# adolfogonzalez3/custom_envs

Hardware: AMD Instinct MI355X
Metric: vectorised env-steps/sec, Optimize-v0 @4096 envs, 1/2/4/8 MI355X vs host CPU (higher is better)
Workload: dtype f64; 1 GPU; Optimize-v0 softmax-regression 256x10 (P=20, obs 41), 4096 envs per GPU, B=N=256, 40-step episodes with in-kernel auto-reset, device-resident actions/outputs; envs_per_gpu=4096, global_envs=4096, n_rows=256, n_features=10, n_classes=2, batch_size=256, steps_per_launch=250, outputs=every step kept: a [250]-record slab per launch, parallelism=env-sharded x1 (no collective)

## Files before the change

custom_envs_amd/csrc/optimize_lr_persist.h:

```cpp
#pragma once

#include "optimize_lr_mfma.h"

namespace ce {

struct ManyArgs {
    int k;
    long long act_stride;
    long long out_step;
};

constexpr int kLpWaves = 4;
constexpr int kLpMaxTpw = 8;

#ifndef CE_LP_G4
#define CE_LP_G4 1
#endif
#ifndef CE_LP_G4_XF
#define CE_LP_G4_XF 1
#endif
#ifndef CE_LP_EPI_SLEEP
#define CE_LP_EPI_SLEEP 0
#endif
#ifndef CE_LP_ROW_PRIO
#define CE_LP_ROW_PRIO 3
#endif
#ifndef CE_LP_LOG_HEAD
#define CE_LP_LOG_HEAD 1
#endif
__host__ __device__ constexpr bool lp_g4(int nkf) { return CE_LP_G4 && nkf <= 3; }

__host__ __device__ constexpr int lp_tpw(int N, int W = kLpWaves) {
    const int per = ((N + 15) / 16 + W - 1) / W;
    return per <= 1 ? 1 : per <= 2 ? 2 : per <= 4 ? 4 : per <= 8 ? 8 : 0;
}
__host__ __device__ constexpr bool lp_pad(int N, int W = kLpWaves) {
    return N % 16 != 0 || (N + 15) / 16 != W * lp_tpw(N, W);
}

#ifdef CE_DIAG
#define LP_STAMP(k)                                                   \
    do {                                                              \
        __builtin_amdgcn_sched_barrier(0);                            \
        lp_st[k] = __builtin_amdgcn_s_memrealtime();                  \
        __builtin_amdgcn_sched_barrier(0);                            \
    } while (0)
#else
#define LP_STAMP(k) \
    do {            \
    } while (0)
#endif

template <int NKF, int TPW, bool PAD, int W>
__global__ __launch_bounds__(kWave * W) void optimize_lr_persist_kernel(StepArgs<double> a, ManyArgs m) {
    constexpr int BLK = kWave * W;
    constexpr int P_MAX = 2 * kLrMaxF;
    constexpr int TD = lr_tile_doubles(NKF);
    constexpr int PR = (kLrEnvs * P_MAX + BLK - 1) / BLK;
    constexpr int OSM = 2 * P_MAX + 4;
    constexpr int NG = TPW < 4 ? TPW : 4;
    __shared__ double red_s[2][W][4][kWave];
    __shared__ double red_l[2][W][kLrEnvs];
    __shared__ double red_h[2][W][kLrEnvs];
    __shared__ __attribute__((aligned(16))) float obs_s[2][kLrEnvs * OSM];
    __shared__ double tab_s[CE_LR_TEXP ? kLrExpTab : 1];

#ifdef CE_DIAG
    unsigned long long lp_st[8] = {0};
#endif
    LP_STAMP(0);
    const int tid = threadIdx.x;
    const int lane = tid & (kWave - 1);
    const int wave = __builtin_amdgcn_readfirstlane(tid >> 6);
    const int c = lane & 15, h = lane >> 4;
    const int E = a.E, F = a.F, P = 2 * F, N = a.N, B = a.B;
    const int OS = a.obs_stride, OL = a.obs_lo;
    const int e0 = blockIdx.x * kLrEnvs;
    const int e = e0 + c;
    const bool env_ok = e < E;
    const unsigned pbase = static_cast<unsigned>(env_ok ? e : 0) * P;
    const double *img = reinterpret_cast<const double *>(a.data);
    const int ntiles = (N + 15) / 16;

#if CE_LR_TEXP
    LrExpSlice<BLK> tslice;
    tslice.load(img + static_cast<unsigned>(ntiles) * TD + kLrMaxF, tid);
#endif
    unsigned ioff[NKF];
    double2 wv[NKF], w0v[NKF];
    float2 av[NKF];
#if CE_LR_NOCLAMP
    double xm[NKF];
    const double *colmax = img + static_cast<unsigned>(ntiles) * TD;
#endif
#pragma unroll
    for (int k = 0; k < NKF; ++k) {
        const int f = 4 * k + h;
        ioff[k] = pbase + (f < F ? 2 * f : 0);
        wv[k] = *reinterpret_cast<const double2 *>(a.W + ioff[k]);
        w0v[k] = *reinterpret_cast<const double2 *>(a.W0 + ioff[k]);
        av[k] = *reinterpret_cast<const float2 *>(a.act + ioff[k]);
#if CE_LR_NOCLAMP
        xm[k] = colmax[f];
#endif
    }
    double xf[TPW][NKF], xg[TPW][4];
    unsigned vmask = 0;
#pragma unroll
    for (int i = 0; i < TPW; ++i) {
        const int t = wave + W * i;
        const bool live = !PAD || t < ntiles;
        const double *ti = img + static_cast<unsigned>(live ? t : 0) * TD;
#pragma unroll
        for (int k = 0; k < NKF; ++k) xf[i][k] = live ? ti[k * kWave + lane] : 0.0;
#pragma unroll
        for (int q = 0; q < 4; ++q) xg[i][q] = live ? ti[(NKF + q) * kWave + lane] : 0.0;
        if constexpr (PAD) {
            const int2 ya = reinterpret_cast<const int2 *>(ti + (NKF + 4) * kWave)[lane];
            const int2 yb = reinterpret_cast<const int2 *>(ti + (NKF + 5) * kWave)[lane];
            const int ys[4] = {ya.x, ya.y, yb.x, yb.y};
#pragma unroll
            for (int q = 0; q < 4; ++q) vmask |= (live && ys[q] >= 0 ? 1u : 0u) << (4 * i + q);
        }
    }
    int step_c = a.step[env_ok ? e : 0];
    const int np_ = kLrEnvs * P;
    const int pmul = (65536 + P - 1) / P;
    int pj[PR], pp[PR], step_p[PR];
    bool prole[PR];
    unsigned gi[PR];
    double g_prev[PR], rG[PR];
#pragma unroll
    for (int r = 0; r < PR; ++r) {
        const int i = tid + r * BLK;
        pj[r] = (i * pmul) >> 16;
        pp[r] = i - pj[r] * P;
        prole[r] = i < np_ && e0 + pj[r] < E;
        gi[r] = static_cast<unsigned>(prole[r] ? e0 + pj[r] : 0) * P + (prole[r] ? pp[r] : 0);
        g_prev[r] = a.G[gi[r]];
        step_p[r] = a.step[prole[r] ? e0 + pj[r] : 0];
    }
    const int sj = tid - (BLK - kLrEnvs);
    const bool srole = sj >= 0 && e0 + sj < E;
    const unsigned es = srole ? e0 + sj : 0;
    double lprev = a.L[es];
    int step_s = a.step[es];
#if CE_LR_TEXP
    tslice.store(tab_s, tid);
    __syncthreads();
#endif
    const double dB = static_cast<double>(B), rB = a.inv_B;
    double rL = rcp_newton2(lprev + 0.1);
#pragma unroll
    for (int r = 0; r < PR; ++r) rG[r] = rcp_newton2(fabs(g_prev[r]) + 1.0);
    if (OL == 0)
        for (int i = tid; i < kLrEnvs * OS; i += BLK) {
            const int j = i / OS, p = i - j * OS;
            if (p < P) obs_s[0][i] = obs_s[1][i] = 0.0f;
        }

    double wd[NKF];
    auto margins = [&]() {
#pragma unroll
        for (int k = 0; k < NKF; ++k) {
            const int f = 4 * k + h;
            const double w0 = wv[k].x - static_cast<double>(av[k].x);
            const double w1 = wv[k].y - static_cast<double>(av[k].y);
            wv[k] = double2{w0, w1};
            wd[k] = f < F ? w0 - w1 : 0.0;
        }
    };
    margins();
#ifdef CE_DIAG
    asm volatile("s_waitcnt vmcnt(0)" ::: "memory");
#endif
    LP_STAMP(1);

    constexpr int QC = 4;
    auto forward = [&](const double (&xv)[NKF]) {
        lr_d4 u = {0.0, 0.0, 0.0, 0.0};
#pragma unroll
        for (int k = 0; k < NKF; ++k) u = __builtin_amdgcn_mfma_f64_16x16x4f64(xv[k], wd[k], u, 0, 0, 0);
        return u;
    };
    const int nenv = E - e0 < kLrEnvs ? E - e0 : kLrEnvs;
    auto flush_obs = [&](int t) {
        float *ob = reinterpret_cast<float *>(reinterpret_cast<char *>(a.obs) + t * m.out_step) +
                    static_cast<unsigned>(e0) * OS;
        const float *src = obs_s[t & 1];
        const int nfl = nenv * OS, n4 = nfl >> 2;
        for (int i = tid; i < n4; i += BLK) {
            typedef float lp_f4 __attribute__((ext_vector_type(4)));
            const lp_f4 v = *reinterpret_cast<const lp_f4 *>(&src[4 * i]);
            asm volatile("global_store_dwordx4 %0, %1, off sc1" ::"v"(ob + 4 * i), "v"(v) : "memory");
        }
        for (int i = 4 * n4 + tid; i < nfl; i += BLK) lr_store(&ob[i], src[i]);
    };

    for (int t = 0; t < m.k; ++t) {
        const int buf = t & 1;
        float2 an[NKF];
        {
            const float *actn = a.act + (t + 1 < m.k ? (t + 1) * m.act_stride : 0);
#pragma unroll
            for (int k = 0; k < NKF; ++k) an[k] = *reinterpret_cast<const float2 *>(actn + ioff[k]);
        }
#if CE_LR_NOCLAMP
        double ub = 0.0;
#pragma unroll
        for (int k = 0; k < NKF; ++k) ub = fma(fabs(wd[k]), xm[k], ub);
        const int tier = lr_tier(ub);
#else
        const int tier = kLrClamped;
#endif
        lr_d4 sacc = {0.0, 0.0, 0.0, 0.0};
        double prod = 1.0, nlog = 0.0, umin = 1.0;
        unsigned miss = 0;
        auto rows = [&](auto tier_c) {
            constexpr int TIER = decltype(tier_c)::value;
#pragma unroll
            for (int g0 = 0; g0 < TPW; g0 += NG) {
                if (g0 > 0) {
                    nlog -= lr_log(prod, tab_s);
                    prod = 1.0;
                }
                lr_d4 u[NG];
#pragma unroll
                for (int i = 0; i < NG; ++i) u[i] = forward(xf[g0 + i]);
#pragma unroll
                for (int i = 0; i < NG; ++i) {
                    double qv[4];
                    static_assert(QC == 4, "the tile's four values go through the exp together");
                    double tx[QC];
                    bool valid[QC];
#pragma unroll
                    for (int j = 0; j < QC; ++j) {
                        if constexpr (TIER == kLrClamped) tx[j] = clamp_u(u[i][j]);
                        else tx[j] = u[i][j];
                        valid[j] = !PAD || ((vmask >> (4 * (g0 + i) + j)) & 1u);
                    }
                    lr_exp_neg<QC>(tx, tab_s);
                    if constexpr (TIER == kLrBatched) {
                        lr_post4(u[i], tx, valid, qv, prod, miss);
                    } else {
#pragma unroll
                        for (int j = 0; j < QC; ++j) lr_post(u[i][j], tx[j], valid[j], qv[j], prod, miss);
                    }
                    lr_tie4<TIER>(u[i], valid, umin);
#pragma unroll
                    for (int q = 0; q < 4; ++q)
                        sacc = __builtin_amdgcn_mfma_f64_16x16x4f64(xg[g0 + i][q], qv[q], sacc, 0, 0, 0);
                }
            }
        };
        lr_run_tier(tier, rows);
        int hits = 4 * TPW - lr_miss_count(miss);
        if (__any(umin < 0x1p-52)) {
#pragma unroll
            for (int i = 0; i < TPW; ++i) {
                const int tt = wave + W * i;
                if (tt >= ntiles) continue;
                const double *ti = img + static_cast<unsigned>(tt) * TD;
                const int2 ya = reinterpret_cast<const int2 *>(ti + (NKF + 4) * kWave)[lane];
                const int2 yb = reinterpret_cast<const int2 *>(ti + (NKF + 5) * kWave)[lane];
                const int yv[4] = {ya.x, ya.y, yb.x, yb.y};
                const lr_d4 uu = forward(xf[i]);
                double tx[4];
#pragma unroll
                for (int q = 0; q < 4; ++q) tx[q] = abs_clamp750(uu[q]);
                exp_neg_multi_clamped<4>(tx);
#pragma unroll
                for (int q = 0; q < 4; ++q)
                    if (yv[q] >= 0 && tx[q] == 1.0) hits += (yv[q] == 0 ? 1 : 0) - lr_hit(uu[q]);
            }
        }
        double lsum = nlog - lr_log(prod, tab_s);
        lsum = fold_pair<16>(lsum, lsum);
        lsum = fold_pair<32>(lsum, lsum);
        const double hsum = static_cast<double>(fold_env_lanes(hits));
#pragma unroll
        for (int r = 0; r < 4; ++r) red_s[buf][wave][r][lane] = sacc[r];
        if (lane < kLrEnvs) {
            red_l[buf][wave][lane] = lsum;
            red_h[buf][wave][lane] = hsum;
        }
        {
            const bool wipe = step_c + 1 >= a.max_steps && a.auto_reset;
            step_c = wipe ? 0 : step_c + 1;
#pragma unroll
            for (int k = 0; k < NKF; ++k)
                if (wipe) wv[k] = w0v[k];
            if (t + 1 < m.k) {
#pragma unroll
                for (int k = 0; k < NKF; ++k) av[k] = an[k];
                margins();
            }
        }
        __syncthreads();
#ifdef CE_DIAG
        if (t == 0) LP_STAMP(2);
        if (t == 1) LP_STAMP(3);
        if (t == m.k - 1) LP_STAMP(4);
#endif
        if (t > 0) flush_obs(t - 1);

        const long long ro = t * m.out_step;
        if (srole) {
            double lt = 0.0, ht = 0.0;
#pragma unroll
            for (int w = 0; w < W; ++w) {
                lt += red_l[buf][w][sj];
                ht += red_h[buf][w][sj];
            }
            const double loss = div_rcp(lt, dB, rB);
            const double acc = div_rcp(ht, dB, rB);
            const double lnew = div_rcp(loss - lprev, lprev + 0.1, rL);
            const int cur = step_s + 1;
            const bool wipe = cur >= a.max_steps && a.auto_reset;
            if (a.reward) lr_store(reinterpret_cast<float *>(reinterpret_cast<char *>(a.reward) + ro) + es,
                                   static_cast<float>(-loss));
            lr_store(reinterpret_cast<float *>(reinterpret_cast<char *>(a.objective) + ro) + es,
                     static_cast<float>(loss));
            lr_store(reinterpret_cast<float *>(reinterpret_cast<char *>(a.accuracy) + ro) + es,
                     static_cast<float>(acc));
            if (a.done) (reinterpret_cast<uint8_t *>(a.done) + ro)[es] = cur >= a.max_steps ? 1 : 0;
            lr_store(reinterpret_cast<int32_t *>(reinterpret_cast<char *>(a.episode_len) + ro) + es, cur);
            obs_s[buf][sj * OS + P - OL] = wipe ? 0.0f : static_cast<float>(lnew);
            lprev = wipe ? 0.0 : lnew;
            step_s = wipe ? 0 : cur;
            rL = rcp_newton2(lprev + 0.1);
        }
#pragma unroll
        for (int r = 0; r < PR; ++r) {
            if (!prole[r]) continue;
            const bool wipe = step_p[r] + 1 >= a.max_steps && a.auto_reset;
            const int f = pp[r] >> 1;
            double sf = 0.0;
#pragma unroll
            for (int w = 0; w < W; ++w) sf += red_s[buf][w][f >> 2][pj[r] + 16 * (f & 3)];
            const double g = div_rcp((pp[r] & 1) ? sf : -sf, dB, rB);
            const double gnew = div_rcp(g, fabs(g_prev[r]) + 1.0, rG[r]);
            obs_s[buf][pj[r] * OS + P + 1 + pp[r] - OL] = wipe ? 0.0f : static_cast<float>(gnew);
            g_prev[r] = wipe ? 0.0 : gnew;
            step_p[r] = wipe ? 0 : step_p[r] + 1;
            rG[r] = rcp_newton2(fabs(g_prev[r]) + 1.0);
        }
    }
    LP_STAMP(5);
    __syncthreads();
    if (m.k > 0) flush_obs(m.k - 1);
    if (wave == 0 && env_ok) {
#pragma unroll
        for (int k = 0; k < NKF; ++k)
            if (4 * k + h < F) {
                lr_store(a.W + ioff[k], wv[k].x);
                lr_store(a.W + ioff[k] + 1, wv[k].y);
            }
    }
#pragma unroll
    for (int r = 0; r < PR; ++r)
        if (prole[r]) lr_store(&a.G[gi[r]], g_prev[r]);
    if (srole) {
        lr_store(&a.L[es], lprev);
        lr_store(&a.step[es], step_s);
    }
#ifdef CE_DIAG
    asm volatile("s_waitcnt vmcnt(0)" ::: "memory");
    LP_STAMP(6);
    const int row = blockIdx.x * W + wave;
    if (row < E && lane < 8) a.diag[static_cast<size_t>(row) * 8 + lane] = lp_st[lane];
#endif
}


template <int NKF, int TPW, bool PAD>
__global__ __launch_bounds__(512) void optimize_lr_persist_ws_kernel(
    double *Wp, const float *actp, const unsigned char *datap, double *Gp, int32_t *stepp, double *Lp,
    unsigned efp, int Np, StepArgs<double> a, ManyArgs m) {
    constexpr int W = 4;
    constexpr int BLK = 512;
    constexpr int EB = BLK - kWave * W;
    constexpr int P_MAX = 2 * kLrMaxF;
    constexpr int TD = lr_tile_doubles(NKF);
    constexpr int PR = (kLrEnvs * P_MAX + EB - 1) / EB;
    constexpr int OSM = 2 * P_MAX + 4;
    constexpr int NG = TPW < 4 ? TPW : 4;
    __shared__ double red_s[2][W][4][kWave];
    __shared__ double red_l[2][W][kLrEnvs];
    __shared__ double red_h[2][W][kLrEnvs];
    __shared__ __attribute__((aligned(16))) float obs_s[2][kLrEnvs * OSM];
    constexpr bool G4 = lp_g4(NKF);
    constexpr int G4S = 14;
    __shared__ __attribute__((aligned(16))) double xgs[G4 ? 1 : W][G4 ? 1 : TPW][4][kWave];
    __shared__ __attribute__((aligned(16))) double xga[G4 ? W : 1][G4 ? TPW : 1][16][G4S];
    __shared__ double tab_s[CE_LR_TEXP ? kLrExpTab : 1];

#ifdef CE_DIAG
    unsigned long long lp_st[8] = {0};
#endif
    LP_STAMP(0);
    const int tid = threadIdx.x;
    const int lane = tid & (kWave - 1);
    const int wave = __builtin_amdgcn_readfirstlane(tid >> 6);
    const int c = lane & 15, h = lane >> 4;
    const int E = static_cast<int>(efp & 0xffffffu), F = static_cast<int>(efp >> 24), P = 2 * F, N = Np, B = a.B;
    const int OS = a.obs_stride, OL = a.obs_lo;
    const int e0 = blockIdx.x * kLrEnvs;
    const double *img = reinterpret_cast<const double *>(datap);
    const int ntiles = (N + 15) / 16;
    const int nenv = E - e0 < kLrEnvs ? E - e0 : kLrEnvs;

#if CE_LR_TEXP
    LrExpSlice<BLK> tslice;
    tslice.load(img + static_cast<unsigned>(ntiles) * TD + kLrMaxF, tid);
#endif
    if (wave < W) {
#if CE_LP_ROW_PRIO > 0
        __builtin_amdgcn_s_setprio(CE_LP_ROW_PRIO);
#endif
        const int e = e0 + c;
        const bool env_ok = e < E;
        const unsigned pbase = static_cast<unsigned>(env_ok ? e : 0) * P;
        unsigned ioff[NKF];
        double2 wv[NKF], w0v[NKF];
        float2 av[NKF];
#if CE_LR_NOCLAMP
        double xm[NKF];
        const double *colmax = img + static_cast<unsigned>(ntiles) * TD;
#endif
#pragma unroll
        for (int k = 0; k < NKF; ++k) {
            const int f = 4 * k + h;
            ioff[k] = pbase + (f < F ? 2 * f : 0);
            wv[k] = *reinterpret_cast<const double2 *>(Wp + ioff[k]);
            av[k] = *reinterpret_cast<const float2 *>(actp + ioff[k]);
#if CE_LR_NOCLAMP
            xm[k] = colmax[f];
#endif
        }
        double xf[TPW][NKF];
#pragma unroll
        for (int k = 0; k < NKF; ++k) w0v[k] = *reinterpret_cast<const double2 *>(a.W0 + ioff[k]);
        unsigned vmask = 0;
#pragma unroll
        for (int i = 0; i < TPW; ++i) {
            const int t = wave + W * i;
            const bool live = !PAD || t < ntiles;
            const double *ti = img + static_cast<unsigned>(live ? t : 0) * TD;
#pragma unroll
            for (int k = 0; k < NKF; ++k) xf[i][k] = live ? ti[k * kWave + lane] : 0.0;
            if constexpr (G4) {
#if CE_LP_G4_XF
                const int km = 4 * (c & 3) + h, j4 = c >> 2;
#pragma unroll
                for (int g = 0; g < NKF; ++g) xga[wave][i][km][j4 * NKF + g] = xf[i][g];
#else
                const int b4 = (lane >> 2) & 3, km = 4 * (lane >> 4) + (lane & 3);
#pragma unroll
                for (int q = 0; q < 4; ++q)
                    if (b4 < NKF) xga[wave][i][km][q * NKF + b4] = live ? ti[(NKF + q) * kWave + lane] : 0.0;
#endif
            } else {
#pragma unroll
                for (int q = 0; q < 4; ++q) xgs[wave][i][q][lane] = live ? ti[(NKF + q) * kWave + lane] : 0.0;
            }
            if constexpr (PAD) {
                const int2 ya = reinterpret_cast<const int2 *>(ti + (NKF + 4) * kWave)[lane];
                const int2 yb = reinterpret_cast<const int2 *>(ti + (NKF + 5) * kWave)[lane];
                const int ys[4] = {ya.x, ya.y, yb.x, yb.y};
#pragma unroll
                for (int q = 0; q < 4; ++q) vmask |= (live && ys[q] >= 0 ? 1u : 0u) << (4 * i + q);
            }
        }
        int step_c = stepp[env_ok ? e : 0];
#if CE_LR_TEXP
        tslice.store(tab_s, tid);
        __syncthreads();
#endif
        double wd[NKF];
        auto margins = [&]() {
#pragma unroll
            for (int k = 0; k < NKF; ++k) {
                const int f = 4 * k + h;
                const double w0 = wv[k].x - static_cast<double>(av[k].x);
                const double w1 = wv[k].y - static_cast<double>(av[k].y);
                wv[k] = double2{w0, w1};
                wd[k] = f < F ? w0 - w1 : 0.0;
            }
        };
        margins();
#ifdef CE_DIAG
        asm volatile("s_waitcnt vmcnt(0)" ::: "memory");
#endif
        LP_STAMP(1);
        constexpr int QC = 4;
        auto forward = [&](const double (&xv)[NKF]) {
            lr_d4 u = {0.0, 0.0, 0.0, 0.0};
#pragma unroll
            for (int k = 0; k < NKF; ++k) u = __builtin_amdgcn_mfma_f64_16x16x4f64(xv[k], wd[k], u, 0, 0, 0);
            return u;
        };
        for (int t = 0; t < m.k; ++t) {
            const int buf = t & 1;
            float2 an[NKF];
            {
                const float *actn = actp + (t + 1 < m.k ? (t + 1) * m.act_stride : 0);
#pragma unroll
                for (int k = 0; k < NKF; ++k) an[k] = *reinterpret_cast<const float2 *>(actn + ioff[k]);
            }
#if CE_LR_NOCLAMP
            double ub = 0.0;
#pragma unroll
            for (int k = 0; k < NKF; ++k) ub = fma(fabs(wd[k]), xm[k], ub);
            const int tier = lr_tier(ub);
#else
            const int tier = kLrClamped;
#endif
            lr_d4 sacc = {0.0, 0.0, 0.0, 0.0};
            double gacc[NKF];
#pragma unroll
            for (int g = 0; g < NKF; ++g) gacc[g] = 0.0;
            double prod = 1.0, nlog = 0.0, umin = 1.0;
            unsigned miss = 0;
            [[maybe_unused]] LrLogHead lhead = {};
            auto rows = [&](auto tier_c) {
                constexpr int TIER = decltype(tier_c)::value;
#pragma unroll
                for (int g0 = 0; g0 < TPW; g0 += NG) {
                    if (g0 > 0) {
                        nlog -= lr_log(prod, tab_s);
                        prod = 1.0;
                    }
                    lr_d4 u[NG];
#pragma unroll
                    for (int i = 0; i < NG; ++i) u[i] = forward(xf[g0 + i]);
#pragma unroll
                    for (int i = 0; i < NG; ++i) {
                        double gv[G4 ? 4 * NKF : 4];
                        if constexpr (G4) {
                            typedef double lp_d2 __attribute__((ext_vector_type(2)));
                            const lp_d2 *src = reinterpret_cast<const lp_d2 *>(
                                &xga[wave][g0 + i][4 * (lane >> 4) + (lane & 3)][0]);
#pragma unroll
                            for (int p2 = 0; p2 < 2 * NKF; ++p2) {
                                const lp_d2 v = src[p2];
                                gv[2 * p2] = v.x;
                                gv[2 * p2 + 1] = v.y;
                            }
                        } else {
#pragma unroll
                            for (int q = 0; q < 4; ++q) gv[q] = xgs[wave][g0 + i][q][lane];
                        }
                        double qv[4];
                        static_assert(QC == 4, "the tile's four values go through the exp together");
                        double tx[QC];
                        bool valid[QC];
#pragma unroll
                        for (int j = 0; j < QC; ++j) {
                            if constexpr (TIER == kLrClamped) tx[j] = clamp_u(u[i][j]);
                            else tx[j] = u[i][j];
                            valid[j] = !PAD || ((vmask >> (4 * (g0 + i) + j)) & 1u);
                        }
                        lr_exp_neg<QC>(tx, tab_s);
                        if constexpr (TIER == kLrBatched) {
                            lr_post4(u[i], tx, valid, qv, prod, miss);
                        } else {
#pragma unroll
                            for (int j = 0; j < QC; ++j)
                                lr_post(u[i][j], tx[j], valid[j], qv[j], prod, miss);
                        }
                        lr_tie4<TIER>(u[i], valid, umin);
#if CE_LP_LOG_HEAD
                        if (g0 + NG >= TPW && i == NG - 1) {
                            lhead = lr_log_head(prod, tab_s);
                            __builtin_amdgcn_sched_barrier(0);
                        }
#endif
                        if constexpr (G4) {
#pragma unroll
                            for (int q = 0; q < 4; ++q)
#pragma unroll
                                for (int g = 0; g < NKF; ++g)
                                    gacc[g] = __builtin_amdgcn_mfma_f64_4x4x4f64(gv[q * NKF + g], qv[q], gacc[g], 0, 0, 0);
                        } else {
#pragma unroll
                            for (int q = 0; q < 4; ++q)
                                sacc = __builtin_amdgcn_mfma_f64_16x16x4f64(gv[q], qv[q], sacc, 0, 0, 0);
                        }
                    }
                }
            };
            lr_run_tier(tier, rows);
            int hits = 4 * TPW - lr_miss_count(miss);
            if (__any(umin < 0x1p-52)) {
#pragma unroll
                for (int i = 0; i < TPW; ++i) {
                    const int tt = wave + W * i;
                    if (tt >= ntiles) continue;
                    const double *ti = img + static_cast<unsigned>(tt) * TD;
                    const int2 ya = reinterpret_cast<const int2 *>(ti + (NKF + 4) * kWave)[lane];
                    const int2 yb = reinterpret_cast<const int2 *>(ti + (NKF + 5) * kWave)[lane];
                    const int yv[4] = {ya.x, ya.y, yb.x, yb.y};
                    const lr_d4 uu = forward(xf[i]);
                    double tx[4];
#pragma unroll
                    for (int q = 0; q < 4; ++q) tx[q] = abs_clamp750(uu[q]);
                    exp_neg_multi_clamped<4>(tx);
#pragma unroll
                    for (int q = 0; q < 4; ++q)
                        if (yv[q] >= 0 && tx[q] == 1.0) hits += (yv[q] == 0 ? 1 : 0) - lr_hit(uu[q]);
                }
            }
#if CE_LP_LOG_HEAD
            double lsum = nlog - lr_log_tail(lhead);
#else
            double lsum = nlog - lr_log(prod, tab_s);
#endif
            lsum = fold_pair<16>(lsum, lsum);
            lsum = fold_pair<32>(lsum, lsum);
            const double hsum = static_cast<double>(fold_env_lanes(hits));
            if constexpr (G4) {
#pragma unroll
                for (int g = 0; g < NKF; ++g) red_s[buf][wave][g][lane] = gacc[g];
            } else {
#pragma unroll
                for (int r = 0; r < 4; ++r) red_s[buf][wave][r][lane] = sacc[r];
            }
            if (lane < kLrEnvs) {
                red_l[buf][wave][lane] = lsum;
                red_h[buf][wave][lane] = hsum;
            }
            {
                const bool wipe = step_c + 1 >= a.max_steps && a.auto_reset;
                step_c = wipe ? 0 : step_c + 1;
                if (__any(wipe)) {
#pragma unroll
                    for (int k = 0; k < NKF; ++k)
                        if (wipe) wv[k] = w0v[k];
                }
                if (t + 1 < m.k) {
#pragma unroll
                    for (int k = 0; k < NKF; ++k) av[k] = an[k];
                    margins();
                }
            }
#ifdef CE_DIAG
            if (t == 1) LP_STAMP(7);
#endif
            __syncthreads();
#ifdef CE_DIAG
            if (t == 0) LP_STAMP(2);
            if (t == 1) LP_STAMP(3);
            if (t == m.k - 1) LP_STAMP(4);
#endif
        }
        LP_STAMP(5);
        __syncthreads();
        if (wave == 0 && env_ok) {
#pragma unroll
            for (int k = 0; k < NKF; ++k)
                if (4 * k + h < F) {
                    lr_store(Wp + ioff[k], wv[k].x);
                    lr_store(Wp + ioff[k] + 1, wv[k].y);
                }
        }
    } else {
        const int te = tid - kWave * W;
        const int np_ = kLrEnvs * P;
        const int pmul = (65536 + P - 1) / P;
        int pj[PR], pp[PR], step_p[PR];
        bool prole[PR];
        unsigned gi[PR];
        double g_prev[PR], rG[PR];
#pragma unroll
        for (int r = 0; r < PR; ++r) {
            const int i = te + r * EB;
            pj[r] = (i * pmul) >> 16;
            pp[r] = i - pj[r] * P;
            prole[r] = i < np_ && e0 + pj[r] < E;
            gi[r] = static_cast<unsigned>(prole[r] ? e0 + pj[r] : 0) * P + (prole[r] ? pp[r] : 0);
            g_prev[r] = Gp[gi[r]];
            step_p[r] = stepp[prole[r] ? e0 + pj[r] : 0];
        }
        const int sj = te - (EB - kLrEnvs);
        const bool srole = sj >= 0 && e0 + sj < E;
        const unsigned es = srole ? e0 + sj : 0;
        double lprev = Lp[es];
        int step_s = stepp[es];
#if CE_LR_TEXP
        tslice.store(tab_s, tid);
#endif
        const double dB = static_cast<double>(B), rB = a.inv_B;
        double rL = rcp_newton2(lprev + 0.1);
#pragma unroll
        for (int r = 0; r < PR; ++r) rG[r] = rcp_newton2(fabs(g_prev[r]) + 1.0);
#if CE_LR_TEXP
        __syncthreads();
#endif
        auto flush_obs = [&](int t) {
            float *ob = reinterpret_cast<float *>(reinterpret_cast<char *>(a.obs) + t * m.out_step) +
                        static_cast<unsigned>(e0) * OS;
            const float *src = obs_s[t & 1];
            const int nfl = nenv * OS, n4 = nfl >> 2;
            for (int i = te; i < n4; i += EB) {
                typedef float lp_f4 __attribute__((ext_vector_type(4)));
                const lp_f4 v = *reinterpret_cast<const lp_f4 *>(&src[4 * i]);
                asm volatile("global_store_dwordx4 %0, %1, off sc1" ::"v"(ob + 4 * i), "v"(v) : "memory");
            }
            for (int i = 4 * n4 + te; i < nfl; i += EB) lr_store(&ob[i], src[i]);
        };
        if (OL == 0)
            for (int i = te; i < kLrEnvs * OS; i += EB) {
                const int j = i / OS, p = i - j * OS;
                if (p < P) obs_s[0][i] = obs_s[1][i] = 0.0f;
            }
        auto epi_steps = [&](auto pow2_c) {
            auto divB = [&](double x) {
                if constexpr (decltype(pow2_c)::value) return x * rB;
                else return div_rcp(x, dB, rB);
            };
            for (int t = 0; t < m.k; ++t) {
                const int buf = t & 1;
                __syncthreads();
#if CE_LP_EPI_SLEEP > 0
                __builtin_amdgcn_s_sleep(CE_LP_EPI_SLEEP);
#endif
    #ifdef CE_DIAG
                if (t == 1) LP_STAMP(2);
    #endif
                if (t > 0) flush_obs(t - 1);
                const long long ro = t * m.out_step;
                if (srole) {
                    double lt = 0.0, ht = 0.0;
    #pragma unroll
                    for (int w = 0; w < W; ++w) {
                        lt += red_l[buf][w][sj];
                        ht += red_h[buf][w][sj];
                    }
                    const double loss = divB(lt);
                    const double acc = divB(ht);
                    const double lnew = div_rcp(loss - lprev, lprev + 0.1, rL);
                    const int cur = step_s + 1;
                    const bool wipe = cur >= a.max_steps && a.auto_reset;
                    if (a.reward) lr_store(reinterpret_cast<float *>(reinterpret_cast<char *>(a.reward) + ro) + es,
                                           static_cast<float>(-loss));
                    lr_store(reinterpret_cast<float *>(reinterpret_cast<char *>(a.objective) + ro) + es,
                             static_cast<float>(loss));
                    lr_store(reinterpret_cast<float *>(reinterpret_cast<char *>(a.accuracy) + ro) + es,
                             static_cast<float>(acc));
                    if (a.done) (reinterpret_cast<uint8_t *>(a.done) + ro)[es] = cur >= a.max_steps ? 1 : 0;
                    lr_store(reinterpret_cast<int32_t *>(reinterpret_cast<char *>(a.episode_len) + ro) + es, cur);
                    float ol = static_cast<float>(lnew);
                    lprev = lnew;
                    step_s = cur;
                    if (__any(wipe)) {
                        if (wipe) {
                            ol = 0.0f;
                            lprev = 0.0;
                            step_s = 0;
                        }
                    }
                    obs_s[buf][sj * OS + P - OL] = ol;
                    rL = rcp_newton2(lprev + 0.1);
                }
    #pragma unroll
                for (int r = 0; r < PR; ++r) {
                    if (!prole[r]) continue;
                    const bool wipe = step_p[r] + 1 >= a.max_steps && a.auto_reset;
                    const int f = pp[r] >> 1;
                    double sf = 0.0;
    #pragma unroll
                    for (int w = 0; w < W; ++w) sf += red_s[buf][w][f >> 2][pj[r] + 16 * (f & 3)];
                    const double g = divB((pp[r] & 1) ? sf : -sf);
                    const double gnew = div_rcp(g, fabs(g_prev[r]) + 1.0, rG[r]);
                    float og = static_cast<float>(gnew);
                    g_prev[r] = gnew;
                    step_p[r] = step_p[r] + 1;
                    if (__any(wipe)) {
                        if (wipe) {
                            og = 0.0f;
                            g_prev[r] = 0.0;
                            step_p[r] = 0;
                        }
                    }
                    obs_s[buf][pj[r] * OS + P + 1 + pp[r] - OL] = og;
                    rG[r] = rcp_newton2(fabs(g_prev[r]) + 1.0);
                }
    #ifdef CE_DIAG
                if (t == 1) {
                    asm volatile("s_waitcnt vmcnt(0) lgkmcnt(0)" ::: "memory");
                    LP_STAMP(7);
                }
    #endif
            }
        };
        if ((B & (B - 1)) == 0) epi_steps(std::true_type{});
        else epi_steps(std::false_type{});
        __syncthreads();
        if (m.k > 0) flush_obs(m.k - 1);
#pragma unroll
        for (int r = 0; r < PR; ++r)
            if (prole[r]) lr_store(&Gp[gi[r]], g_prev[r]);
        if (srole) {
            lr_store(&Lp[es], lprev);
            lr_store(&stepp[es], step_s);
        }
    }
#ifdef CE_DIAG
    asm volatile("s_waitcnt vmcnt(0)" ::: "memory");
    LP_STAMP(6);
    const int row = blockIdx.x * 8 + wave;
    if (row < E && lane < 8) a.diag[static_cast<size_t>(row) * 8 + lane] = lp_st[lane];
#endif
}

}
```

Before: 1.785 billion env-steps/s.

## Hand weight-margin update to an epilogue wave via an LDS ring

Moves the per-step weight update (action subtraction, auto-reset wipe, margin/tier computation and final weight writeback) out of the four MFMA row waves into a dedicated epilogue wave. That wave precomputes wd and tier two steps ahead and passes them through a two-slot shared-memory ring. The row waves then only read wd from LDS each step, taking action loads and reset logic off their critical path. In exchange it adds LDS traffic and an extra barrier, and correctness now depends on the ring depth matching the per-step __syncthreads cadence.

```diff
diff --git a/custom_envs_amd/csrc/optimize_lr_persist.h b/custom_envs_amd/csrc/optimize_lr_persist.h
--- a/custom_envs_amd/csrc/optimize_lr_persist.h
+++ b/custom_envs_amd/csrc/optimize_lr_persist.h
@@ -28,7 +28,12 @@
 #ifndef CE_LP_LOG_HEAD
 #define CE_LP_LOG_HEAD 1
 #endif
+#ifndef CE_LP_WD_HANDOVER
+#define CE_LP_WD_HANDOVER 1
+#endif
 __host__ __device__ constexpr bool lp_g4(int nkf) { return CE_LP_G4 && nkf <= 3; }
+constexpr int kLpWdWave = 2;
+constexpr int kLpWdRing = 2;
 
 __host__ __device__ constexpr int lp_tpw(int N, int W = kLpWaves) {
     const int per = ((N + 15) / 16 + W - 1) / W;
@@ -394,6 +399,10 @@
     __shared__ __attribute__((aligned(16))) double xgs[G4 ? 1 : W][G4 ? 1 : TPW][4][kWave];
     __shared__ __attribute__((aligned(16))) double xga[G4 ? W : 1][G4 ? TPW : 1][16][G4S];
     __shared__ double tab_s[CE_LR_TEXP ? kLrExpTab : 1];
+#if CE_LP_WD_HANDOVER
+    __shared__ double wd_s[kLpWdRing][NKF][kWave];
+    __shared__ int tier_s[kLpWdRing];
+#endif
 
 #ifdef CE_DIAG
     unsigned long long lp_st[8] = {0};
@@ -418,6 +427,7 @@
 #if CE_LP_ROW_PRIO > 0
         __builtin_amdgcn_s_setprio(CE_LP_ROW_PRIO);
 #endif
+#if !CE_LP_WD_HANDOVER
         const int e = e0 + c;
         const bool env_ok = e < E;
         const unsigned pbase = static_cast<unsigned>(env_ok ? e : 0) * P;
@@ -438,9 +448,12 @@
             xm[k] = colmax[f];
 #endif
         }
+#endif
         double xf[TPW][NKF];
+#if !CE_LP_WD_HANDOVER
 #pragma unroll
         for (int k = 0; k < NKF; ++k) w0v[k] = *reinterpret_cast<const double2 *>(a.W0 + ioff[k]);
+#endif
         unsigned vmask = 0;
 #pragma unroll
         for (int i = 0; i < TPW; ++i) {
@@ -472,12 +485,19 @@
                 for (int q = 0; q < 4; ++q) vmask |= (live && ys[q] >= 0 ? 1u : 0u) << (4 * i + q);
             }
         }
+#if !CE_LP_WD_HANDOVER
         int step_c = stepp[env_ok ? e : 0];
+#endif
 #if CE_LR_TEXP
         tslice.store(tab_s, tid);
+#endif
+#if CE_LR_TEXP || CE_LP_WD_HANDOVER
         __syncthreads();
 #endif
         double wd[NKF];
+#if CE_LP_WD_HANDOVER
+        int slot = 0;
+#else
         auto margins = [&]() {
 #pragma unroll
             for (int k = 0; k < NKF; ++k) {
@@ -489,6 +509,7 @@
             }
         };
         margins();
+#endif
 #ifdef CE_DIAG
         asm volatile("s_waitcnt vmcnt(0)" ::: "memory");
 #endif
@@ -502,6 +523,16 @@
         };
         for (int t = 0; t < m.k; ++t) {
             const int buf = t & 1;
+#if CE_LP_WD_HANDOVER
+#pragma unroll
+            for (int k = 0; k < NKF; ++k) wd[k] = wd_s[slot][k][lane];
+#if CE_LR_NOCLAMP
+            const int tier = __builtin_amdgcn_readfirstlane(tier_s[slot]);
+#else
+            const int tier = kLrClamped;
+#endif
+            slot = slot == kLpWdRing - 1 ? 0 : slot + 1;
+#else
             float2 an[NKF];
             {
                 const float *actn = actp + (t + 1 < m.k ? (t + 1) * m.act_stride : 0);
@@ -515,6 +546,7 @@
             const int tier = lr_tier(ub);
 #else
             const int tier = kLrClamped;
+#endif
 #endif
             lr_d4 sacc = {0.0, 0.0, 0.0, 0.0};
             double gacc[NKF];
@@ -630,6 +662,7 @@
                 red_l[buf][wave][lane] = lsum;
                 red_h[buf][wave][lane] = hsum;
             }
+#if !CE_LP_WD_HANDOVER
             {
                 const bool wipe = step_c + 1 >= a.max_steps && a.auto_reset;
                 step_c = wipe ? 0 : step_c + 1;
@@ -644,6 +677,7 @@
                     margins();
                 }
             }
+#endif
 #ifdef CE_DIAG
             if (t == 1) LP_STAMP(7);
 #endif
@@ -656,6 +690,7 @@
         }
         LP_STAMP(5);
         __syncthreads();
+#if !CE_LP_WD_HANDOVER
         if (wave == 0 && env_ok) {
 #pragma unroll
             for (int k = 0; k < NKF; ++k)
@@ -664,6 +699,7 @@
                     lr_store(Wp + ioff[k] + 1, wv[k].y);
                 }
         }
+#endif
     } else {
         const int te = tid - kWave * W;
         const int np_ = kLrEnvs * P;
@@ -687,6 +723,76 @@
         const unsigned es = srole ? e0 + sj : 0;
         double lprev = Lp[es];
         int step_s = stepp[es];
+#if CE_LP_WD_HANDOVER
+        const bool wown = wave == W + kLpWdWave;
+        const int e = e0 + c;
+        const bool env_ok = e < E;
+        unsigned ioff[NKF];
+        double2 wv[NKF], w0v[NKF];
+        float2 an[NKF];
+        [[maybe_unused]] double xm[NKF];
+        int step_c = 0;
+        auto wd_wipe = [&]() {
+            const bool wipe = step_c + 1 >= a.max_steps && a.auto_reset;
+            step_c = wipe ? 0 : step_c + 1;
+            if (__any(wipe)) {
+#pragma unroll
+                for (int k = 0; k < NKF; ++k)
+                    if (wipe) wv[k] = w0v[k];
+            }
+        };
+        auto wd_emit = [&](int slot, const float2 (&av)[NKF]) {
+            double wd[NKF];
+#pragma unroll
+            for (int k = 0; k < NKF; ++k) {
+                const int f = 4 * k + h;
+                const double w0 = wv[k].x - static_cast<double>(av[k].x);
+                const double w1 = wv[k].y - static_cast<double>(av[k].y);
+                wv[k] = double2{w0, w1};
+                wd[k] = f < F ? w0 - w1 : 0.0;
+            }
+#if CE_LR_NOCLAMP
+            double ub = 0.0;
+#pragma unroll
+            for (int k = 0; k < NKF; ++k) ub = fma(fabs(wd[k]), xm[k], ub);
+            tier_s[slot] = lr_tier(ub);
+#endif
+#pragma unroll
+            for (int k = 0; k < NKF; ++k) wd_s[slot][k][lane] = wd[k];
+        };
+        auto act_load = [&](int s, float2 (&av)[NKF]) {
+            const float *acts = actp + s * m.act_stride;
+#pragma unroll
+            for (int k = 0; k < NKF; ++k) av[k] = *reinterpret_cast<const float2 *>(acts + ioff[k]);
+        };
+        if (wown) {
+            const unsigned pbase = static_cast<unsigned>(env_ok ? e : 0) * P;
+#if CE_LR_NOCLAMP
+            const double *colmax = img + static_cast<unsigned>(ntiles) * TD;
+#endif
+#pragma unroll
+            for (int k = 0; k < NKF; ++k) {
+                const int f = 4 * k + h;
+                ioff[k] = pbase + (f < F ? 2 * f : 0);
+                wv[k] = *reinterpret_cast<const double2 *>(Wp + ioff[k]);
+                w0v[k] = *reinterpret_cast<const double2 *>(a.W0 + ioff[k]);
+#if CE_LR_NOCLAMP
+                xm[k] = colmax[f];
+#endif
+            }
+            step_c = stepp[env_ok ? e : 0];
+            float2 a0[kLpWdRing][NKF];
+#pragma unroll
+            for (int s = 0; s < kLpWdRing; ++s)
+                if (s < m.k) act_load(s, a0[s]);
+            if (kLpWdRing < m.k) act_load(kLpWdRing, an);
+#pragma unroll
+            for (int s = 0; s < kLpWdRing; ++s) {
+                if (s > 0 && s <= m.k) wd_wipe();
+                if (s < m.k) wd_emit(s, a0[s]);
+            }
+        }
+#endif
 #if CE_LR_TEXP
         tslice.store(tab_s, tid);
 #endif
@@ -694,7 +800,7 @@
         double rL = rcp_newton2(lprev + 0.1);
 #pragma unroll
         for (int r = 0; r < PR; ++r) rG[r] = rcp_newton2(fabs(g_prev[r]) + 1.0);
-#if CE_LR_TEXP
+#if CE_LR_TEXP || CE_LP_WD_HANDOVER
         __syncthreads();
 #endif
         auto flush_obs = [&](int t) {
@@ -719,6 +825,9 @@
                 if constexpr (decltype(pow2_c)::value) return x * rB;
                 else return div_rcp(x, dB, rB);
             };
+#if CE_LP_WD_HANDOVER
+            int wslot = 0;
+#endif
             for (int t = 0; t < m.k; ++t) {
                 const int buf = t & 1;
                 __syncthreads();
@@ -728,6 +837,19 @@
     #ifdef CE_DIAG
                 if (t == 1) LP_STAMP(2);
     #endif
+#if CE_LP_WD_HANDOVER
+                if (wown && t + kLpWdRing <= m.k) {
+                    wd_wipe();
+                    if (t + kLpWdRing < m.k) {
+                        float2 av[NKF];
+    #pragma unroll
+                        for (int k = 0; k < NKF; ++k) av[k] = an[k];
+                        if (t + kLpWdRing + 1 < m.k) act_load(t + kLpWdRing + 1, an);
+                        wd_emit(wslot, av);
+                    }
+                }
+                wslot = wslot == kLpWdRing - 1 ? 0 : wslot + 1;
+#endif
                 if (t > 0) flush_obs(t - 1);
                 const long long ro = t * m.out_step;
                 if (srole) {
@@ -805,6 +927,16 @@
             lr_store(&Lp[es], lprev);
             lr_store(&stepp[es], step_s);
         }
+#if CE_LP_WD_HANDOVER
+        if (wown && env_ok) {
+#pragma unroll
+            for (int k = 0; k < NKF; ++k)
+                if (4 * k + h < F) {
+                    lr_store(Wp + ioff[k], wv[k].x);
+                    lr_store(Wp + ioff[k] + 1, wv[k].y);
+                }
+        }
+#endif
     }
 #ifdef CE_DIAG
     asm volatile("s_waitcnt vmcnt(0)" ::: "memory");
```

After: 1.833 billion env-steps/s (median of 6 runs). Within noise of the previous version (+2.6%).
